# Kamino666/Video-Captioning-Transformer

Hardware: AMD Instinct MI355X
Metric: video-caption train samples/sec (whole node) (higher is better)
Workload: dtype bf16; 1 GPU; configs[1]: 2 enc + 2 dec layers d=512 ff=2048 H=8 V=30522, synthetic (256,12,512) features -> 20-token captions per GPU, fwd+bwd+Adam, dropout 0.3, SCE alpha 0.5; global_batch=256, per_gpu_batch=256, seq_len=20, frames=12, parallelism=dp1, executor=list

## Files before the change

### video-captioning-transformer_amd/csrc/vct_common.h

```cpp
#pragma once
#include <hip/hip_runtime.h>
#include <stdint.h>
#include <utility>
#include <type_traits>
#include "../../include/vct_hip.h"
#include "vct_runtime.h"

namespace vct {

typedef __attribute__((ext_vector_type(4))) uint32_t stream_u32x4;
typedef __attribute__((ext_vector_type(2))) uint32_t stream_u32x2;
__device__ __forceinline__ void store_stream16(void* dst, const stream_u32x4 v) {
  asm volatile("global_store_dwordx4 %0, %1, off sc1" :: "v"(dst), "v"(v) : "memory");
}
__device__ __forceinline__ void store_stream8(void* dst, const stream_u32x2 v) {
  asm volatile("global_store_dwordx2 %0, %1, off sc1" :: "v"(dst), "v"(v) : "memory");
}


typedef __attribute__((ext_vector_type(8))) __bf16 bf16x8;
typedef __attribute__((ext_vector_type(4))) __bf16 bf16x4;
typedef __attribute__((ext_vector_type(4))) short s16x4;
typedef __attribute__((ext_vector_type(8))) short s16x8;
typedef __attribute__((ext_vector_type(4))) float f32x4;
// ... 68 lines not shown
}

struct Dropout {
  uint32_t key;
  uint32_t thresh;
  float scale;
  bool on;
};
__device__ __forceinline__ Dropout make_dropout(const uint32_t* seed, uint32_t site, float p) {
  Dropout d;
  d.on = (seed != nullptr) && (p > 0.0f);
  d.key = d.on ? (seed[0] * 0x9E3779B1u) ^ (site * 0x85EBCA77u + 0x165667B1u) : 0u;
  d.thresh = d.on ? (uint32_t)fminf(p * 65536.0f + 0.5f, 65535.0f) : 0u;
  d.scale = d.on ? 1.0f / (1.0f - p) : 1.0f;
  return d;
}
__device__ __forceinline__ uint32_t hash32(uint32_t x) {
  x ^= x >> 16; x *= 0x85EBCA6Bu; x ^= x >> 13; x *= 0xC2B2AE35u; x ^= x >> 16;
  return x;
}
__device__ __forceinline__ float drop_mult(const Dropout& d, uint32_t idx) {
  if (!d.on) return 1.0f;
  const uint32_t h = hash32(((idx >> 1) * 0x9E3779B1u) ^ d.key);
  const uint32_t f = (idx & 1u) ? (h >> 16) : (h & 0xffffu);
  return f < d.thresh ? 0.0f : d.scale;
}
template <int N> __device__ __forceinline__ void drop_mults(const Dropout& d, uint32_t idx, float (&m)[N]) {
  static_assert(N % 2 == 0, "pairs");
  if (!d.on) {
#pragma unroll
    for (int j = 0; j < N; j++) m[j] = 1.0f;
    return;
  }
  if ((idx & 1u) == 0u) {
#pragma unroll
    for (int k = 0; k < N / 2; k++) {
      const uint32_t h = hash32((((idx >> 1) + (uint32_t)k) * 0x9E3779B1u) ^ d.key);
      m[2 * k] = (h & 0xffffu) < d.thresh ? 0.0f : d.scale;
      m[2 * k + 1] = (h >> 16) < d.thresh ? 0.0f : d.scale;
    }
  } else {
#pragma unroll
    for (int j = 0; j < N; j++) m[j] = drop_mult(d, idx + (uint32_t)j);
  }
}

__device__ __forceinline__ float wave_sum(float v) {
#pragma unroll
  for (int o = 32; o > 0; o >>= 1) v += __shfl_xor(v, o);
  return v;
}
__device__ __forceinline__ float wave_max(float v) {
#pragma unroll
  for (int o = 32; o > 0; o >>= 1) v = fmaxf(v, __shfl_xor(v, o));
  return v;
}
template <int NW> __device__ __forceinline__ float block_sum(float v, float* red) {
  v = wave_sum(v);
  const int w = threadIdx.x >> 6, l = threadIdx.x & 63;
  __syncthreads();
  if (l == 0) red[w] = v;
  __syncthreads();
  float s = 0.0f;
#pragma unroll
  for (int i = 0; i < NW; i++) s += red[i];
  return s;
}
template <int NW> __device__ __forceinline__ float block_max(float v, float* red) {
  v = wave_max(v);
  const int w = threadIdx.x >> 6, l = threadIdx.x & 63;
  __syncthreads();
  if (l == 0) red[w] = v;
  __syncthreads();
  float s = red[0];
#pragma unroll
  for (int i = 1; i < NW; i++) s = fmaxf(s, red[i]);
  return s;
}

__device__ __forceinline__ s16x4 lds_tr16(const bf16_t* p) {
  return __builtin_amdgcn_ds_read_tr16_b64_v4i16((__attribute__((address_space(3))) s16x4*)(p));
}

template <class F, int... Is>
__device__ __forceinline__ void static_for_impl(F&& f, std::integer_sequence<int, Is...>) {
  (f(std::integral_constant<int, Is>{}), ...);
}
template <int N, class F> __device__ __forceinline__ void static_for(F&& f) {
  static_for_impl(static_cast<F&&>(f), std::make_integer_sequence<int, N>{});
}

template <typename T> struct DTypeOf;
template <> struct DTypeOf<float> { static constexpr int v = VCT_F32; };
template <> struct DTypeOf<bf16_t> { static constexpr int v = VCT_BF16; };

}

#define VCT_CHECK_LAUNCH()                               \
  do {                                                   \
    hipError_t e__ = hipGetLastError();                  \
    if (e__ != hipSuccess) return (int)e__;              \
  } while (0)
```

### video-captioning-transformer_amd/csrc/vct_gemm.hip

```cpp
#include <cstdlib>
#include <cstring>
#include "vct_common.h"
#include "vct_gemm_params.h"

namespace vct {

template <typename TI> struct GemmCfg;
template <> struct GemmCfg<float> { static constexpr int BK = 16, VEC = 4, KPAD = 4; };

struct alignas(16) Vec16 { uint32_t w[4]; };
__device__ __forceinline__ Vec16 vec_zero() { Vec16 v; v.w[0] = v.w[1] = v.w[2] = v.w[3] = 0u; return v; }

template <typename TI, bool MC, int R>
struct Stager {
  using Cfg = GemmCfg<TI>;
  static constexpr int BK = Cfg::BK, VEC = Cfg::VEC;
  static constexpr bool BF = sizeof(TI) == 2;
  static constexpr int NV = (R * BK / VEC) / 256;
  static constexpr int KC_STRIDE = BK + Cfg::KPAD;
  static constexpr int LDS_ELEMS = R * KC_STRIDE;
  static_assert(NV >= 1, "tile too small for 256 threads");

  __device__ __forceinline__ static void load(Vec16 (&regs)[NV], const TI* __restrict__ base, long ld, int r0,
                                              int r_ext, int k0, int K) {
// ... 166 lines not shown
      for (int q = 0; q < VO; q += 4) {
        const f32x4 t = *reinterpret_cast<const f32x4*>(stg + rr * STG_STRIDE + cc + q);
        v[q] = t[0]; v[q + 1] = t[1]; v[q + 2] = t[2]; v[q + 3] = t[3];
      }
      if (row >= p.M || col >= p.N) return;
      const bool full = vec_ok && (col + VO <= p.N);
      if (part) {
        float* dst = partC + (size_t)row * p.N + col;
        if (full) {
#pragma unroll
          for (int q = 0; q < VO; q += 4) *reinterpret_cast<f32x4*>(dst + q) = f32x4{v[q], v[q + 1], v[q + 2], v[q + 3]};
        } else {
          for (int q = 0; q < VO; q++) if (col + q < p.N) dst[q] = v[q];
        }
        return;
      }
      if (full) {
        OutV dv, av, ov, pv;
        const bool has_d = dact != nullptr, has_a = addend != nullptr;
        if (has_d) dv = *reinterpret_cast<const OutV*>(dact + (size_t)row * p.ld_dact + col);
        if (has_a) av = *reinterpret_cast<const OutV*>(addend + (size_t)row * p.ld_addend + col);
#pragma unroll
        for (int q = 0; q < VO; q++) {
          float x = v[q] + bvec[c][q];
          pv.e[q] = from_f<TO>(x);
          x = act_f(p.act, x);
          if (has_d) x *= dact_f(p.dact_kind, to_f<TO>(dv.e[q]));
          x *= drop_mult(dr, (uint32_t)row * (uint32_t)p.N + (uint32_t)(col + q));
          if (has_a) x += to_f<TO>(av.e[q]);
          ov.e[q] = from_f<TO>(x);
        }
        *reinterpret_cast<OutV*>(C + (size_t)row * p.ldc + col) = ov;
        if (preact != nullptr) {
          if ((p.ld_preact % VO) == 0) *reinterpret_cast<OutV*>(preact + (size_t)row * p.ld_preact + col) = pv;
          else for (int q = 0; q < VO; q++) preact[(size_t)row * p.ld_preact + col + q] = pv.e[q];
        }
      } else {
        for (int q = 0; q < VO; q++) {
          if (col + q >= p.N) break;
          float x = v[q] + bvec[c][q];
          if (preact != nullptr) preact[(size_t)row * p.ld_preact + col + q] = from_f<TO>(x);
          x = act_f(p.act, x);
          if (dact != nullptr) x *= dact_f(p.dact_kind, to_f<TO>(dact[(size_t)row * p.ld_dact + col + q]));
          x *= drop_mult(dr, (uint32_t)row * (uint32_t)p.N + (uint32_t)(col + q));
          if (addend != nullptr) x += to_f<TO>(addend[(size_t)row * p.ld_addend + col + q]);
          C[(size_t)row * p.ldc + col + q] = from_f<TO>(x);
        }
      }
    });
  });
}

template <typename TO>
__global__ void splitk_reduce_kernel(const float* __restrict__ partial, TO* __restrict__ C, long ldc, int M, int N,
                                     int S, const float* __restrict__ bias_partial, float* __restrict__ bias_grad) {
  const size_t total = (size_t)M * N;
  for (size_t idx = (size_t)blockIdx.x * blockDim.x + threadIdx.x; idx < total; idx += (size_t)gridDim.x * blockDim.x) {
    float s = 0.0f;
    for (int z = 0; z < S; z++) s += partial[(size_t)z * total + idx];
    const int row = (int)(idx / N), col = (int)(idx % N);
    C[(size_t)row * ldc + col] = from_f<TO>(s);
  }
  if (bias_grad != nullptr) {
    for (int row = blockIdx.x * blockDim.x + threadIdx.x; row < M; row += gridDim.x * blockDim.x) {
      float s = 0.0f;
      for (int z = 0; z < S; z++) s += bias_partial[(size_t)z * M + row];
      bias_grad[row] = s;
    }
  }
}

struct Plan { int bm, bn, nbuf, waves8; int split; int tiles_m, tiles_n, nkt, kt_per; };

static bool gemm_can_split(const vct_gemm_desc* d) {
  return d->bias == nullptr && d->act == VCT_ACT_NONE && d->preact == nullptr &&
         d->addend == nullptr && d->dact_src == nullptr && !(d->seed != nullptr && d->p_drop > 0.0f);
}

static bool use_counters(const vct_gemm_desc* d, const Plan& pl) {
  const int64_t partial_bytes = (int64_t)pl.split * d->M * d->N * 4;
  return d->tile_counters != nullptr && d->dtype == VCT_BF16 && (long)pl.tiles_m * pl.tiles_n <= (long)d->n_tile_counters &&
         partial_bytes <= ((int64_t)16 << 20);
}
static Plan gemm_plan(const vct_gemm_desc* d, bool have_ws) {
  Plan pl;
  pl.nbuf = 2;
  pl.waves8 = 0;
  const bool bf = d->dtype == VCT_BF16;
  const int BK = bf ? 64 : 16;
  pl.nkt = (d->K + BK - 1) / BK;
  auto tiles = [&](int bm, int bn) { return (long)((d->M + bm - 1) / bm) * ((d->N + bn - 1) / bn); };
  if (bf) {
    static const int cand[7][2] = {{128, 128}, {128, 64}, {64, 128}, {64, 64}, {256, 128}, {320, 128}, {64, 128}};
    int pick = 3;
    const int rsv = d->reserved >= 99 ? 0 : d->reserved;
    const int tsel = rsv % 10;
    pl.nbuf = (rsv / 10) ? (rsv / 10) : 2;
    const bool cover_ok = d->out_dtype == VCT_BF16 && d->ta == 0;
    if (tsel == 5) { pick = 0; pl.waves8 = 1; }
    else if (tsel == 8) { pick = 1; pl.waves8 = 4; }
    else if (tsel == 6 && cover_ok) { pick = 4; pl.waves8 = 6; pl.nbuf = 2; }
    else if (tsel == 7 && cover_ok) { pick = 5; pl.waves8 = 7; pl.nbuf = 2; }
    else if (tsel == 9 && cover_ok) { pick = 6; pl.waves8 = 9; pl.nbuf = 2; }
    else if (tsel >= 1 && tsel <= 4) pick = tsel - 1;
    else {
      pick = 3;
      static const bool legacy = getenv("VCT_GEMM_4WAVE_ONLY") != nullptr;
      if ((pl.nkt >= 64 && tiles(128, 128) >= 128) || (tiles(64, 64) >= 16384 && d->N >= 4096)) {
        pick = 0; pl.waves8 = legacy ? 0 : 1;
        if (legacy && pl.nkt < 64) pick = 2;
      } else if (!legacy && d->N >= 1024 && d->M >= 2048 && pl.nkt <= 16) { pick = 1; pl.waves8 = 4; }
    }
    pl.bm = cand[pick][0]; pl.bn = cand[pick][1];
  } else {
    pl.bm = pl.bn = (tiles(128, 128) >= 384) ? 128 : 64;
  }
  pl.tiles_m = (d->M + pl.bm - 1) / pl.bm;
  pl.tiles_n = (d->N + pl.bn - 1) / pl.bn;
  const long nt = (long)pl.tiles_m * pl.tiles_n;
  int split = 1;
  if (d->split_k > 1) split = d->split_k;
  else if (d->split_k == 0 && nt < 384 && pl.nkt >= 8) split = (int)((767 + nt) / nt);
  const bool epilogue = !gemm_can_split(d);
  if (!have_ws || (epilogue && (d->tile_counters == nullptr || !bf))) split = 1;
  if (epilogue && d->split_k == 0 && d->M > 16) split = 1;
  if (split > pl.nkt / 2) split = pl.nkt / 2 > 0 ? pl.nkt / 2 : 1;
  if (split < 1) split = 1;
  pl.kt_per = (pl.nkt + split - 1) / split;
  pl.split = (pl.nkt + pl.kt_per - 1) / pl.kt_per;
  if ((epilogue || d->adam != nullptr) && pl.split > 1 && !use_counters(d, pl)) { pl.split = 1; pl.kt_per = pl.nkt; }
  return pl;
}

template <typename TI, typename TO, int TA, int TB, int BM>
static void launch_gemm(const GemmP& p, dim3 grid, hipStream_t st) {
  vct::launch((gemm_kernel<TI, TO, TA, TB, BM, BM>), grid, dim3(256), 0, st, p);
}

template <typename TI, typename TO>
static int dispatch_layout(const vct_gemm_desc* d, const GemmP& p, int bm, dim3 grid, hipStream_t st) {
  const int key = d->ta * 2 + d->tb;
#define VCT_L(TA_, TB_)                                              \
  if (bm == 128) launch_gemm<TI, TO, TA_, TB_, 128>(p, grid, st);    \
  else launch_gemm<TI, TO, TA_, TB_, 64>(p, grid, st);               \
  return VCT_OK;
  switch (key) {
    case 1: { VCT_L(0, 1) }
    case 0: { VCT_L(0, 0) }
    case 2: { VCT_L(1, 0) }
    default: return VCT_E_SHAPE;
  }
#undef VCT_L
}

int gemm_bf16_v2_dispatch(const vct_gemm_desc* d, const GemmP& p, int bm, int bn, int nbuf, dim3 grid, hipStream_t st);
int gemm256_try(const vct_gemm_desc* d, hipStream_t st, bool* used, int* reduce_split);
int gemm_skinny_try(const vct_gemm_desc* d, hipStream_t st, bool* used);
int gemm_pt_try(const vct_gemm_desc* d, hipStream_t st, bool* used);

}

using namespace vct;

static int64_t ws_bytes(const vct_gemm_desc* d, const Plan& pl) {
  if (pl.split <= 1) return 0;
  return (int64_t)pl.split * ((int64_t)d->M * d->N + d->M) * 4;
}

extern "C" int64_t vct_gemm_workspace_bytes(const vct_gemm_desc* d) {
  if (d == nullptr) return 0;
  return ws_bytes(d, gemm_plan(d, true));
}

static int check_desc(const vct_gemm_desc* d) {
  if (d == nullptr || d->A == nullptr || d->B == nullptr || d->C == nullptr) return VCT_E_ARG;
  if (d->dtype != VCT_F32 && d->dtype != VCT_BF16) return VCT_E_ARG;
  if (d->out_dtype != VCT_F32 && d->out_dtype != VCT_BF16) return VCT_E_ARG;
  if (d->M <= 0 || d->N <= 0 || d->K <= 0) return VCT_E_SHAPE;
  if (d->ta == 1 && d->tb == 1) return VCT_E_SHAPE;
  const int vec = d->dtype == VCT_BF16 ? 8 : 4;
  if (d->lda % vec || d->ldb % vec) return VCT_E_ALIGN;
  if (((uintptr_t)d->A & 15) || ((uintptr_t)d->B & 15)) return VCT_E_ALIGN;
  if (d->dact_src != nullptr && d->act == VCT_ACT_NONE) return VCT_E_ARG;
  if (d->bias_grad != nullptr && d->dtype == VCT_BF16 && !(d->ta == 1 && d->tb == 0 && d->out_dtype == VCT_F32)) return VCT_E_ARG;
  if (d->adam != nullptr) {
    const vct_gemm_adam* a = d->adam;
    if (!(d->dtype == VCT_BF16 && d->out_dtype == VCT_F32 && d->ta == 1 && d->tb == 0)) return VCT_E_ARG;
    if (d->bias != nullptr || d->act != VCT_ACT_NONE || d->preact != nullptr || d->addend != nullptr || d->dact_src != nullptr ||
        (d->seed != nullptr && d->p_drop > 0.0f))
      return VCT_E_ARG;
    if (!a->param || !a->exp_avg || !a->exp_avg_sq || !a->hyper || !a->step) return VCT_E_ARG;
    if (((uintptr_t)a->param | (uintptr_t)a->exp_avg | (uintptr_t)a->exp_avg_sq | (uintptr_t)d->C) & 15) return VCT_E_ALIGN;
    if (d->ldc % 4) return VCT_E_ALIGN;
    if (a->shadow != nullptr && (((uintptr_t)a->shadow & 7) || (a->ld_shadow % 4))) return VCT_E_ALIGN;
    if (a->pk_stream != nullptr && (a->shadow == nullptr || ((uintptr_t)a->pk_stream & 15) || a->pk_K < d->N || (a->pk_K % 8) ||
                                    a->pk_row0 < 0 || (a->pk_mode != 0 && a->pk_mode != 1)))
      return VCT_E_ARG;
    if (a->pk_stream != nullptr)
      for (int i = 0; i < 4; i++) if (a->pk_chunk0[i] >= 0xffff) return VCT_E_ARG;
  }
  return VCT_OK;
}

static void fill_params(const vct_gemm_desc* d, const Plan& pl, GemmP& p) {
  p.A = d->A; p.B = d->B; p.C = d->C;
  p.lda = d->lda; p.ldb = d->ldb; p.ldc = d->ldc;
  p.M = d->M; p.N = d->N; p.K = d->K;
  p.kt_per_split = pl.kt_per;
  p.tiles_m = pl.tiles_m;
  p.tiles_n = pl.tiles_n;
  p.act = d->dact_src != nullptr ? VCT_ACT_NONE : d->act;
  p.dact_kind = d->dact_src != nullptr ? d->act : VCT_ACT_NONE;
  p.bias = d->bias;
  p.preact = d->preact; p.ld_preact = d->ld_preact;
  p.addend = d->addend; p.ld_addend = d->ld_addend;
  p.dact = d->dact_src; p.ld_dact = d->ld_dact;
  p.seed = d->seed; p.site = d->site; p.p_drop = d->p_drop;
  p.bias_grad = d->bias_grad;
  p.partial = nullptr; p.bias_partial = nullptr; p.counters = nullptr;
  memset(&p.adam, 0, sizeof(p.adam));
  if (d->adam != nullptr) {
    const vct_gemm_adam* a = d->adam;
    p.adam.param = a->param; p.adam.m = a->exp_avg; p.adam.v = a->exp_avg_sq;
    p.adam.shadow = reinterpret_cast<uint16_t*>(a->shadow); p.adam.ld_shadow = (long)a->ld_shadow;
    p.adam.pk_stream = reinterpret_cast<uint16_t*>(a->pk_stream); p.adam.pk_K = a->pk_K; p.adam.pk_mode = a->pk_mode;
    {
      auto f = [](int c) { return (unsigned long long)(c < 0 || c >= 0xffff ? 0xffff : c); };
      p.adam.pk_chunks = f(a->pk_chunk0[0]) | (f(a->pk_chunk0[1]) << 16) | (f(a->pk_chunk0[2]) << 32) | (f(a->pk_chunk0[3]) << 48);
    }
    p.adam.pk_row0 = a->pk_row0; p.adam.store_grad = a->store_grad;
    p.adam.hyper = a->hyper; p.adam.step = a->step;
  }
  p.waves8 = pl.waves8;
  p.split = pl.split;
  {
    static const char* env = getenv("VCT_GEMM_NT");
    p.nt_store = env != nullptr ? atoi(env) : 0;
  }
  {
    static const char* env = getenv("VCT_GEMM_NT_PREACT");
    p.nt_preact = env != nullptr ? (env[0] == '1') : 0;
  }
  {
    static const char* env = getenv("VCT_GEMM_ORDER");
    const int ts = pl.tiles_m < pl.tiles_n ? pl.tiles_m : pl.tiles_n;
    p.short_fast = env != nullptr ? (env[0] == '1') : (pl.split > 1 && ts <= 4);
  }
  if (pl.split > 1) {
    if (use_counters(d, pl)) p.counters = d->tile_counters;
    p.partial = reinterpret_cast<float*>(d->workspace);
    p.bias_partial = p.partial + (size_t)pl.split * d->M * d->N;
  }
}

extern "C" int vct_gemm(const vct_gemm_desc* d, void* stream) {
  const int ok = check_desc(d);
  if (ok != VCT_OK) return ok;
  hipStream_t st = (hipStream_t)stream;
  const bool general_only = d->adam != nullptr;
  if (!general_only) {
    bool used = false;
    const int rcs = gemm_skinny_try(d, st, &used);
    if (rcs != VCT_OK || used) return rcs;
  }
  if (!general_only || (d->ta == 1 && d->tb == 0)) {
    bool used = false;
    int rsplit = 1;
    const int rc256 = gemm256_try(d, st, &used, &rsplit);
    if (rc256 != VCT_OK) return rc256;
    if (used) {
      if (rsplit > 1) {
        const size_t total = (size_t)d->M * d->N;
        const int blocks = (int)((total + 255) / 256 < 2048 ? (total + 255) / 256 : 2048);
        vct::launch((splitk_reduce_kernel<bf16_t>), dim3(blocks), dim3(256), 0, st, reinterpret_cast<const float*>(d->workspace),
                    reinterpret_cast<bf16_t*>(d->C), (long)d->ldc, d->M, d->N, rsplit, (const float*)nullptr, (float*)nullptr);
        VCT_CHECK_LAUNCH();
      }
      return VCT_OK;
    }
  }

  if (!general_only) {
    bool used = false;
    const int rcp = gemm_pt_try(d, st, &used);
    if (rcp != VCT_OK || used) return rcp;
  }

  const int64_t need = vct_gemm_workspace_bytes(d);
  const bool have_ws = d->workspace != nullptr && d->workspace_bytes >= need && need > 0;
  if (d->split_k > 1 && !have_ws) return VCT_E_WORKSPACE;
  const Plan pl = gemm_plan(d, have_ws);

  GemmP p;
  fill_params(d, pl, p);
  const dim3 grid(pl.tiles_m * pl.tiles_n, 1, pl.split);
  int rc;
  if (d->dtype == VCT_BF16) {
    rc = gemm_bf16_v2_dispatch(d, p, pl.bm, pl.bn, pl.nbuf, grid, st);
  } else {
    if (d->out_dtype != VCT_F32) return VCT_E_ARG;
    rc = dispatch_layout<float, float>(d, p, pl.bm, grid, st);
  }
  if (rc != VCT_OK) return rc;
  VCT_CHECK_LAUNCH();
  if (pl.split > 1 && p.counters == nullptr) {
    const size_t total = (size_t)d->M * d->N;
    const int blocks = (int)((total + 255) / 256 < 2048 ? (total + 255) / 256 : 2048);
    if (d->out_dtype == VCT_F32)
      vct::launch((splitk_reduce_kernel<float>), dim3(blocks), dim3(256), 0, st, p.partial,
                         reinterpret_cast<float*>(d->C), (long)d->ldc, d->M, d->N, pl.split, p.bias_partial, d->bias_grad);
    else
      vct::launch((splitk_reduce_kernel<bf16_t>), dim3(blocks), dim3(256), 0, st, p.partial,
                         reinterpret_cast<bf16_t*>(d->C), (long)d->ldc, d->M, d->N, pl.split, p.bias_partial, d->bias_grad);
    VCT_CHECK_LAUNCH();
  }
  return VCT_OK;
}

namespace vct {
int gemm_bf16_v2_grouped_tn(const GemmGroupP& g, int bm, int bn, int total_wg, hipStream_t st);
}

struct GroupTile { int bm, bn, waves8; };
static long group_tiles(const vct_gemm_desc* descs, int n, const GroupTile& t) {
  long gt = 0;
  for (int k = 0; k < n; k++) gt += (long)((descs[k].M + t.bm - 1) / t.bm) * ((descs[k].N + t.bn - 1) / t.bn);
  return gt;
}
static GroupTile grouped_tile(const vct_gemm_desc* descs, int n) {
  static const int env_sel = [] { const char* e = getenv("VCT_GROUP_TILE"); return e ? atoi(e) : 0; }();
  const int sel = descs[0].reserved % 10 ? descs[0].reserved % 10 : env_sel;
  if (sel == 4) return GroupTile{64, 64, 0};
  if (sel == 8) return GroupTile{128, 64, 4};
  if (sel == 5) return GroupTile{128, 128, 1};
  const GroupTile big{128, 128, 1};
  return group_tiles(descs, n, big) >= 160 ? big : GroupTile{64, 64, 0};
}
static Plan grouped_plan(const vct_gemm_desc* d, const GroupTile& t, long gt) {
  Plan pl;
  pl.bm = t.bm; pl.bn = t.bn; pl.nbuf = 2; pl.waves8 = t.waves8;
  pl.nkt = (d->K + 63) / 64;
  pl.tiles_m = (d->M + t.bm - 1) / t.bm;
  pl.tiles_n = (d->N + t.bn - 1) / t.bn;
  int split = gt >= 192 ? 1 : (int)((255 + gt) / gt);
  if (d->split_k >= 1) split = d->split_k;
  if (split > pl.nkt / 4) split = pl.nkt / 4 > 0 ? pl.nkt / 4 : 1;
  while (split > 1 && (int64_t)split * d->M * d->N * 4 > ((int64_t)16 << 20)) split--;
  if (split < 1) split = 1;
  pl.kt_per = (pl.nkt + split - 1) / split;
  pl.split = (pl.nkt + pl.kt_per - 1) / pl.kt_per;
  return pl;
}

extern "C" int64_t vct_gemm_grouped_workspace_bytes(const vct_gemm_desc* descs, int32_t n, int32_t i) {
  if (descs == nullptr || n < 1 || n > VCT_GEMM_GROUP_MAX || i < 0 || i >= n) return 0;
  const GroupTile t = grouped_tile(descs, n);
  return ws_bytes(descs + i, grouped_plan(descs + i, t, group_tiles(descs, n, t)));
}

extern "C" int vct_gemm_grouped(const vct_gemm_desc* descs, int32_t n, void* stream) {
  if (descs == nullptr || n < 1 || n > VCT_GEMM_GROUP_MAX) return VCT_E_ARG;
  for (int i = 0; i < n; i++) {
    const vct_gemm_desc* d = descs + i;
    const int ok = check_desc(d);
    if (ok != VCT_OK) return ok;
    if (d->dtype != VCT_BF16 || d->out_dtype != VCT_F32 || d->ta != 1 || d->tb != 0 || !gemm_can_split(d)) return VCT_E_ARG;
  }
  const GroupTile t = grouped_tile(descs, n);
  const long gt = group_tiles(descs, n, t);
  GemmGroupP g;
  g.n = n;
  int wg = 0;
  static const bool group_map_on = [] { const char* e = getenv("VCT_GROUP_MAP"); return !(e && e[0] == '0'); }();
  bool group_map = group_map_on;
  for (int i = 0; i < n && group_map; i++) group_map = grouped_plan(descs + i, t, gt).split == 1;
  for (int i = 0; i < n; i++) {
    const vct_gemm_desc* d = descs + i;
    const Plan pl = grouped_plan(d, t, gt);
    if (pl.split > 1) {
      if (!use_counters(d, pl)) return VCT_E_WORKSPACE;
      if (d->workspace == nullptr || d->workspace_bytes < ws_bytes(d, pl)) return VCT_E_WORKSPACE;
    }
    fill_params(d, pl, g.p[i]);
    g.start[i] = wg;
    wg += group_map ? pl.tiles_m * pl.tiles_n : (pl.tiles_m * pl.tiles_n * pl.split + 7) & ~7;
  }
  g.total = group_map ? wg : 0;
  for (int i = n; i < VCT_GEMM_GROUP_MAX; i++) { g.start[i] = wg; g.p[i] = g.p[0]; }
  wg = (wg + 7) & ~7;
  const int rc = gemm_bf16_v2_grouped_tn(g, t.bm, t.bn, wg, (hipStream_t)stream);
  if (rc != VCT_OK) return rc;
  VCT_CHECK_LAUNCH();
  return VCT_OK;
}
```

### video-captioning-transformer_amd/csrc/vct_gemm_bf16_kernel.h

```cpp
#pragma once
#include <type_traits>
#ifndef VCT_GEMM_DMA_IL
#define VCT_GEMM_DMA_IL(TA, TB, BM, BN, NW) ((TA) == 0 && (TB) == 0)
#endif
#include "vct_common.h"
#include "vct_adam_core.h"
#include "vct_gemm_params.h"

namespace vct {

constexpr int BK2 = 64;

__device__ __forceinline__ int kc_off(int row, int chunk) { return row * 128 + ((chunk ^ (row & 7)) << 4); }
template <int R> __device__ __forceinline__ int mc_off(int krow, int col) {
  constexpr int NB = R / 16;
  const int b = col >> 4;
  return krow * (R * 2) + (((b ^ (krow & (NB - 1))) << 5) | ((col & 15) << 1));
}

template <bool MC, int R, int NW>
__device__ __forceinline__ void dma_tile(unsigned char* lds, const bf16_t* __restrict__ base, long ld, int r0, int r_ext,
                                         int k0, int wave, int lane) {
  constexpr int NI = R * 8 / (64 * NW);
  static_assert(NI >= 1, "tile too small for this many waves");
// ... 190 lines not shown

  const bf16_t* A = reinterpret_cast<const bf16_t*>(p.A);
  const bf16_t* B = reinterpret_cast<const bf16_t*>(p.B);

  f32x4 acc[TM][TN];
  constexpr int TMB = (TM + WGN - 1) / WGN;
  f32x4 accb[TMB];
#pragma unroll
  for (int u = 0; u < TMB; u++) accb[u] = f32x4{0, 0, 0, 0};
#pragma unroll
  for (int i = 0; i < TM; i++) {
#pragma unroll
    for (int j = 0; j < TN; j++) acc[i][j] = f32x4{0, 0, 0, 0};
  }
  constexpr bool BG = (TA == 1 && TB == 0 && sizeof(TO) == 4);
  const bool do_bias_grad = BG && (p.bias_grad != nullptr) && (tile_n == 0);
  const s16x8 ones_s = {0x3F80, 0x3F80, 0x3F80, 0x3F80, 0x3F80, 0x3F80, 0x3F80, 0x3F80};
  const bf16x8 ones = __builtin_bit_cast(bf16x8, ones_s);

  auto compute = [&](const unsigned char* la, const unsigned char* lb, auto WITH_DMA, unsigned char* nb, const int ktn) {
    constexpr bool DMA = decltype(WITH_DMA)::value;
    constexpr int KS = BK2 / 32;
    bf16x8 fa[KS][TM], fb[KS][TN];
#pragma unroll
    for (int ks = 0; ks < KS; ks++) {
#pragma unroll
      for (int i = 0; i < TM; i++) fa[ks][i] = frag2<A_MC, BM, KSPLIT>(la, wm * WM + i * 16, ks, lane);
#pragma unroll
      for (int j = 0; j < TN; j++) fb[ks][j] = frag2<B_MC, BN, KSPLIT>(lb, wn * WN + j * 16, ks, lane);
    }
#pragma unroll
    for (int ks = 0; ks < KS; ks++)
#pragma unroll
      for (int i = 0; i < TM; i++)
#pragma unroll
        for (int j = 0; j < TN; j++) acc[i][j] = __builtin_amdgcn_mfma_f32_16x16x32_bf16(fa[ks][i], fb[ks][j], acc[i][j], 0, 0, 0);
    constexpr int N_DSREAD = KS * (TM * (A_MC ? 2 : 1) + TN * (B_MC ? 2 : 1));
    constexpr int NMF = KS * TM * TN;
    if constexpr (DMA) {
      constexpr int NP = BM * 8 / (64 * NW) + BN * 8 / (64 * NW);
      constexpr int GRP = (NMF / 2 / NP) > 0 ? (NMF / 2 / NP) : 1;
      dma_tile<A_MC, BM, NW>(nb, A, p.lda, m0, p.M, ktn * BK2, wave, lane);
      dma_tile<B_MC, BN, NW>(nb + A_BYTES, B, p.ldb, n0, p.N, ktn * BK2, wave, lane);
      __builtin_amdgcn_sched_group_barrier(0x100, N_DSREAD, 0);
      static_for<NP>([&](auto) {
        __builtin_amdgcn_sched_group_barrier(0x008, GRP, 0);
        __builtin_amdgcn_sched_group_barrier(0x020, 1, 0);
      });
      if constexpr (NMF - NP * GRP > 0) __builtin_amdgcn_sched_group_barrier(0x008, NMF - NP * GRP, 0);
    } else {
      __builtin_amdgcn_sched_group_barrier(0x100, N_DSREAD, 0);
      __builtin_amdgcn_sched_group_barrier(0x008, NMF, 0);
    }
    if constexpr (BG) {
      if (do_bias_grad) {
        static_for<TM>([&](auto I) {
          constexpr int i = decltype(I)::value;
          if (wn == i % WGN) {
#pragma unroll
            for (int ks = 0; ks < KS; ks++) accb[i / WGN] = __builtin_amdgcn_mfma_f32_16x16x32_bf16(fa[ks][i], ones, accb[i / WGN], 0, 0, 0);
          }
        });
      }
    }
  };

  auto stage = [&](int kt, int buf) {
    unsigned char* nb = lds_raw + buf * BUF_BYTES;
    if (kt < kt_full_end) {
      dma_tile<A_MC, BM, NW>(nb, A, p.lda, m0, p.M, kt * BK2, wave, lane);
      dma_tile<B_MC, BN, NW>(nb + A_BYTES, B, p.ldb, n0, p.N, kt * BK2, wave, lane);
    } else {
      tail_tile<A_MC, BM, NT>(nb, A, p.lda, m0, p.M, kt * BK2, p.K, tid);
      tail_tile<B_MC, BN, NT>(nb + A_BYTES, B, p.ldb, n0, p.N, kt * BK2, p.K, tid);
    }
  };
  if constexpr (NBUF == 1) {
    for (int kt = kt_begin; kt < kt_end; kt++) {
      if (kt > kt_begin) __syncthreads();
      stage(kt, 0);
      __syncthreads();
      compute(lds_raw, lds_raw + A_BYTES, std::false_type{}, nullptr, 0);
    }
  } else {
    static_assert(NBUF == 2, "NBUF is 1 or 2");
    if (kt_begin < kt_end) stage(kt_begin, 0);
    int cur = 0;
    int kt = kt_begin;
    if constexpr (DMA_IL) {
      for (; kt + 1 < kt_full_end; kt++) {
        __syncthreads();
        const unsigned char* la = lds_raw + cur * BUF_BYTES;
        compute(la, la + A_BYTES, std::true_type{}, lds_raw + (cur ^ 1) * BUF_BYTES, kt + 1);
        cur ^= 1;
      }
    }
    for (; kt < kt_end; kt++) {
      __syncthreads();
      if (kt + 1 < kt_end) stage(kt + 1, cur ^ 1);
      compute(lds_raw + cur * BUF_BYTES, lds_raw + cur * BUF_BYTES + A_BYTES, std::false_type{}, nullptr, 0);
      cur ^= 1;
    }
  }

  const int c16 = lane & 15, g4 = (lane >> 4) * 4;
  if (do_bias_grad && c16 == 0) {
    float* bg = p.partial != nullptr ? p.bias_partial + (size_t)zid * p.M : p.bias_grad;
#pragma unroll
    for (int u = 0; u < TMB; u++)
#pragma unroll
      for (int r = 0; r < 4; r++) {
        const int i = wn + u * WGN;
        const int row = m0 + wm * WM + i * 16 + g4 + r;
        if (i < TM && row < p.M) {
          if (p.counters != nullptr) coherent_store1(bg + row, accb[u][r]);
          else bg[row] = accb[u][r];
        }
      }
  }
  __syncthreads();
  float* stage_base = reinterpret_cast<float*>(lds_raw);
  constexpr int VO = 16 / (int)sizeof(TO);
  constexpr bool SLAB = (BM * BN != 128 * 128);
  constexpr int SLAB_ROWS = WGM * 16, CPRW = BN / VO;
  constexpr int CPRV = WN / VO;
  constexpr int SSTR = SLAB ? BN + 4 : WN + 4;
  constexpr int STAGE_FLOATS = SLAB ? SLAB_ROWS * SSTR : NW * 16 * SSTR;
  constexpr int NSLAB = (SLAB && 2 * STAGE_FLOATS * 4 <= NBUF * BUF_BYTES) ? 2 : 1;
  static_assert(STAGE_FLOATS * 4 <= NBUF * BUF_BYTES, "epilogue staging must fit in the operand buffers");
  static_assert(!SLAB || (SLAB_ROWS * CPRW) % NT == 0, "slab chunks must divide over the workgroup");
  constexpr int CPL = SLAB ? SLAB_ROWS * CPRW / NT : (16 * CPRV + 63) / 64;
  const bool part = p.partial != nullptr;
  int e_lds[CPL], e_row[CPL], e_col[CPL];
  bool e_act[CPL];
  float bvec[CPL][VO];
#pragma unroll
  for (int c = 0; c < CPL; c++) {
    if constexpr (SLAB) {
      const int chunk = c * NT + tid;
      const int sr = chunk / CPRW, sc = (chunk % CPRW) * VO;
      e_lds[c] = sr * SSTR + sc; e_row[c] = (sr >> 4) * WM + (sr & 15); e_col[c] = sc; e_act[c] = true;
    } else {
      const int chunk = c * 64 + lane;
      const int rr = (chunk / CPRV) & 15, cc = (chunk % CPRV) * VO;
      e_lds[c] = wave * 16 * SSTR + rr * SSTR + cc; e_row[c] = wm * WM + rr; e_col[c] = wn * WN + cc;
      e_act[c] = chunk < 16 * CPRV;
    }
#pragma unroll
    for (int q = 0; q < VO; q++) bvec[c][q] = 0.0f;
  }
  if (p.bias != nullptr && (!part || p.counters != nullptr)) {
#pragma unroll
    for (int c = 0; c < CPL; c++) {
#pragma unroll
      for (int q = 0; q < VO; q++) bvec[c][q] = p.bias[min(n0 + e_col[c] + q, p.N - 1)];
    }
  }

  const Dropout dr = make_dropout(p.seed, p.site, p.p_drop);
  TO* C = reinterpret_cast<TO*>(p.C);
  TO* preact = reinterpret_cast<TO*>(p.preact);
  const TO* addend = reinterpret_cast<const TO*>(p.addend);
  const TO* dact = reinterpret_cast<const TO*>(p.dact);
  float* partC = part ? p.partial + (size_t)zid * (size_t)p.M * (size_t)p.N : nullptr;
  const long ldo = part ? (long)p.N : p.ldc;
  const bool vec_ok = (ldo % VO == 0) && (part || (((uintptr_t)p.C & 15) == 0));
// ... 160 lines not shown
      const int row = m0 + e_row[c] + i * 16, col = n0 + e_col[c];
      float v[VO];
#pragma unroll
      for (int q = 0; q < VO; q += 4) {
        const f32x4 t = *reinterpret_cast<const f32x4*>(stage + e_lds[c] + q);
        v[q] = t[0]; v[q + 1] = t[1]; v[q + 2] = t[2]; v[q + 3] = t[3];
      }
      if (!e_act[c]) return;
      if (row >= p.M || col >= p.N) return;
      const bool full = vec_ok && (col + VO <= p.N);
      if (part) {
        float* dst = partC + (size_t)row * p.N + col;
        if (p.counters != nullptr) {
          if (full) {
#pragma unroll
            for (int q = 0; q < VO; q += 2) coherent_store2(dst + q, v[q], v[q + 1]);
          } else {
            for (int q = 0; q < VO; q++) if (col + q < p.N) coherent_store1(dst + q, v[q]);
          }
        } else if (full) {
#pragma unroll
          for (int q = 0; q < VO; q += 4) *reinterpret_cast<f32x4*>(dst + q) = f32x4{v[q], v[q + 1], v[q + 2], v[q + 3]};
        } else {
          for (int q = 0; q < VO; q++) if (col + q < p.N) dst[q] = v[q];
        }
        return;
      }
      finish(row, col, v, bvec[c], full, adam_direct ? &areg[c] : nullptr);
    });
  });

  if (part && p.counters != nullptr) {
    __shared__ int s_last;
    asm volatile("s_waitcnt vmcnt(0)" ::: "memory");
    __syncthreads();
    if (tid == 0)
      s_last = (__hip_atomic_fetch_add(p.counters + wgid, 1, __ATOMIC_RELAXED, __HIP_MEMORY_SCOPE_AGENT) == p.split - 1) ? 1 : 0;
    __syncthreads();
    if (!s_last) return;
    const size_t zstride = (size_t)p.M * (size_t)p.N;
    static_for<TM>([&](auto I) {
      constexpr int i = decltype(I)::value;
      static_for<CPL>([&](auto CI) {
        constexpr int c = decltype(CI)::value;
        const int row = m0 + e_row[c] + i * 16, col = n0 + e_col[c];
        if (!e_act[c] || row >= p.M || col >= p.N) return;
        const float* src = p.partial + (size_t)row * p.N + col;
        const bool full = vec_ok && (col + VO <= p.N) && (p.ldc % VO == 0) && (((uintptr_t)p.C & 15) == 0);
        float s[VO];
#pragma unroll
        for (int q = 0; q < VO; q++) s[q] = 0.0f;
        if (full) {
          for (int z = 0; z < p.split; z++) {
#pragma unroll
            for (int q = 0; q < VO; q += 2) {
              float t0, t1;
              coherent_load2(src + (size_t)z * zstride + q, t0, t1);
              s[q] += t0; s[q + 1] += t1;
            }
          }
        } else {
          for (int q = 0; q < VO; q++) {
            if (col + q >= p.N) break;
            for (int z = 0; z < p.split; z++) s[q] += coherent_load1(src + (size_t)z * zstride + q);
          }
        }
        finish(row, col, s, bvec[c], full, nullptr);
      });
    });
    if (p.bias_grad != nullptr && tile_n == 0) {
      for (int r = tid; r < BM; r += NT) {
        const int row = m0 + r;
        if (row < p.M) {
          float a = 0.0f;
          for (int z = 0; z < p.split; z++) a += coherent_load1(p.bias_partial + (size_t)z * p.M + row);
          p.bias_grad[row] = a;
        }
      }
    }
    if (tid == 0) __hip_atomic_store(p.counters + wgid, 0, __ATOMIC_RELAXED, __HIP_MEMORY_SCOPE_AGENT);
  }
}

constexpr int gemm_min_waves(int bm, int bn, int nw) { return nw == 8 ? (bm * bn == 128 * 128 ? 4 : (bm * bn == 128 * 64 ? 6 : 1)) : 1; }

template <typename TO, int TA, int TB, int BM, int BN, int NBUF, int WGM = 2, int WGN = 2>
__global__ __launch_bounds__(64 * WGM * WGN, gemm_min_waves(BM, BN, WGM * WGN)) void gemm_bf16_v2_kernel(const GemmP p) {
  gemm_bf16_v2_body<TO, TA, TB, BM, BN, NBUF, WGM, WGN>(p, blockIdx.x, blockIdx.z);
}

template <typename TO, int TA, int TB, int BM, int BN, int NBUF, int WGM, int WGN>
__global__ __launch_bounds__(64 * WGM * WGN, gemm_min_waves(BM, BN, WGM * WGN)) void gemm_bf16_v2_grouped_kernel(const GemmGroupP g) {
  const int b = blockIdx.x;
  int at = b;
  const bool direct = g.total > 0;
  if (direct) {
    const int xcd = b & 7, slot = b >> 3;
    const int q = g.total >> 3, r = g.total & 7;
    if (slot >= q + (xcd < r ? 1 : 0)) return;
    at = (xcd < r ? xcd * (q + 1) : r * (q + 1) + (xcd - r) * q) + slot;
  }
  int gi = 0;
#pragma unroll
  for (int i = 1; i < VCT_GEMM_GROUP_MAX; i++) gi = (i < g.n && at >= g.start[i]) ? i : gi;
  const GemmP& p = g.p[gi];
  const int local = at - g.start[gi], nwg = p.tiles_m * p.tiles_n;
  if (local >= nwg * p.split) return;
  gemm_bf16_v2_body<TO, TA, TB, BM, BN, NBUF, WGM, WGN>(p, local % nwg, local / nwg, direct);
}

template <typename TO, int TA, int TB, int NBUF>
static int launch_tiles(const GemmP& p, int bm, int bn, dim3 grid, hipStream_t st) {
#define VCT_LAUNCH(BM_, BN_) vct::launch((gemm_bf16_v2_kernel<TO, TA, TB, BM_, BN_, NBUF>), grid, dim3(256), 0, st, p)
  if (p.waves8) {
#define VCT_LW(BM_, BN_, WM_, WN_) vct::launch((gemm_bf16_v2_kernel<TO, TA, TB, BM_, BN_, NBUF, WM_, WN_>), grid, dim3(64 * WM_ * WN_), 0, st, p)
    if (p.waves8 == 1 && bm == 128 && bn == 128) VCT_LW(128, 128, 2, 4);
    else if (p.waves8 == 4 && bm == 128 && bn == 64) VCT_LW(128, 64, 4, 2);
    else if constexpr (sizeof(TO) == 2 && TA == 0 && NBUF == 2) {
      if (p.waves8 == 6 && bm == 256 && bn == 128) VCT_LW(256, 128, 4, 2);
      else if (p.waves8 == 7 && bm == 320 && bn == 128) VCT_LW(320, 128, 4, 2);
      else if (p.waves8 == 9 && bm == 64 && bn == 128) VCT_LW(64, 128, 2, 4);
      else return VCT_E_SHAPE;
    }
    else return VCT_E_SHAPE;
#undef VCT_LW
  }
  else if (bm == 128 && bn == 128) VCT_LAUNCH(128, 128);
  else if (bm == 128 && bn == 64) VCT_LAUNCH(128, 64);
  else if (bm == 64 && bn == 128) VCT_LAUNCH(64, 128);
  else if (bm == 64 && bn == 64) VCT_LAUNCH(64, 64);
  else return VCT_E_SHAPE;
#undef VCT_LAUNCH
  return VCT_OK;
}

template <typename TO, int TA, int TB>
static int launch_nbuf(const GemmP& p, int bm, int bn, int nbuf, dim3 grid, hipStream_t st) {
  if (nbuf == 1) return launch_tiles<TO, TA, TB, 1>(p, bm, bn, grid, st);
  return launch_tiles<TO, TA, TB, 2>(p, bm, bn, grid, st);
}


template <int TA, int TB>
static int gemm_bf16_v2_layout(const vct_gemm_desc* d, const GemmP& p, int bm, int bn, int nbuf, dim3 grid, hipStream_t st) {
  return d->out_dtype == VCT_BF16 ? launch_nbuf<bf16_t, TA, TB>(p, bm, bn, nbuf, grid, st)
                                  : launch_nbuf<float, TA, TB>(p, bm, bn, nbuf, grid, st);
}

}
```

### video-captioning-transformer_amd/csrc/vct_gemm_bf16_tn.hip

```cpp
#include "vct_gemm_bf16_kernel.h"
namespace vct {
int gemm_bf16_v2_tn(const vct_gemm_desc* d, const GemmP& p, int bm, int bn, int nbuf, dim3 grid, hipStream_t st) {
  return gemm_bf16_v2_layout<1, 0>(d, p, bm, bn, nbuf, grid, st);
}
int gemm_bf16_v2_grouped_tn(const GemmGroupP& g, int bm, int bn, int total_wg, hipStream_t st) {
  if (bm == 128 && bn == 128)
    vct::launch((gemm_bf16_v2_grouped_kernel<float, 1, 0, 128, 128, 2, 2, 4>), dim3(total_wg), dim3(512), 0, st, g);
  else if (bm == 128 && bn == 64)
    vct::launch((gemm_bf16_v2_grouped_kernel<float, 1, 0, 128, 64, 2, 4, 2>), dim3(total_wg), dim3(512), 0, st, g);
  else if (bm == 64 && bn == 64)
    vct::launch((gemm_bf16_v2_grouped_kernel<float, 1, 0, 64, 64, 2, 2, 2>), dim3(total_wg), dim3(256), 0, st, g);
  else
    return VCT_E_SHAPE;
  return VCT_OK;
}
}
```

### video-captioning-transformer_amd/csrc/vct_gemm_params.h

```cpp
#pragma once
#include <stdint.h>
#include "../../include/vct_hip.h"

namespace vct {

struct AdamEpiP {
  float* param; float* m; float* v;
  uint16_t* shadow; long ld_shadow;
  uint16_t* pk_stream; int pk_K, pk_mode; int pk_row0; int store_grad;
  unsigned long long pk_chunks;
  const float* hyper; const int32_t* step;
};

struct GemmP {
  const void* A; const void* B; void* C;
  long lda, ldb, ldc;
  int M, N, K;
  int kt_per_split;
  int tiles_m, tiles_n;
  int act;
  int dact_kind;
  const float* bias;
  void* preact; long ld_preact;
  const void* addend; long ld_addend;
  const void* dact; long ld_dact;
  const uint32_t* seed; uint32_t site; float p_drop;
  float* bias_grad;
  float* partial;
  float* bias_partial;
  int waves8;
  int split;
  int* counters;
  int nt_store;
  int nt_preact;
  int short_fast;
  AdamEpiP adam;
};

struct GemmGroupP {
  int n;
  int total;
  int start[VCT_GEMM_GROUP_MAX];
  GemmP p[VCT_GEMM_GROUP_MAX];
};

}
```

Measured before the change: 123,500 samples/s.

## Add three-slot LDS ring pipeline for selected bf16 GEMM shapes

Adds an NBUF=3 main loop to the bf16 GEMM kernel. Global-to-LDS staging runs two k-tiles ahead, LDS fragment reads use inline asm with immediate offsets, and explicit vmcnt/lgkmcnt waits let the second k-step's reads overlap the first k-step's MFMAs. The planner switches the default-enabled form (mask 2: NN bf16 64x64 tiles with kt_per >= 4) to the ring, and the grouped TN path can opt in through a mask. The ring uses more LDS per block and lowers launch-bounds occupancy hints, so fewer blocks may fit per CU. An env-controlled dynamic-LDS padding probe is also added, off by default.

```diff
diff --git a/video-captioning-transformer_amd/csrc/vct_common.h b/video-captioning-transformer_amd/csrc/vct_common.h
--- a/video-captioning-transformer_amd/csrc/vct_common.h
+++ b/video-captioning-transformer_amd/csrc/vct_common.h
@@ -174,6 +174,28 @@
   return __builtin_amdgcn_ds_read_tr16_b64_v4i16((__attribute__((address_space(3))) s16x4*)(p));
 }
 
+template <int OFF> __device__ __forceinline__ s16x4 lds_tr16_asm(uint32_t ad) {
+  static_assert(OFF >= 0 && OFF < 65536, "ds offset field is 16 bits");
+  s16x4 v;
+  asm volatile("ds_read_b64_tr_b16 %0, %1 offset:%2" : "=v"(v) : "v"(ad), "n"(OFF) : "memory");
+  return v;
+}
+template <int OFF> __device__ __forceinline__ s16x8 lds_b128_asm(uint32_t ad) {
+  static_assert(OFF >= 0 && OFF < 65536, "ds offset field is 16 bits");
+  s16x8 v;
+  asm volatile("ds_read_b128 %0, %1 offset:%2" : "=v"(v) : "v"(ad), "n"(OFF) : "memory");
+  return v;
+}
+template <typename V> __device__ __forceinline__ void lds_asm_tie(V& v) { asm volatile("" : "+v"(v)); }
+template <int N> __device__ __forceinline__ void wait_vmcnt() {
+  static_assert(N >= 0 && N < 64, "vmcnt is 6 bits");
+  asm volatile("s_waitcnt vmcnt(%0)" :: "n"(N) : "memory");
+}
+template <int N> __device__ __forceinline__ void wait_lgkmcnt() {
+  static_assert(N >= 0 && N < 16, "lgkmcnt is 4 bits");
+  asm volatile("s_waitcnt lgkmcnt(%0)" :: "n"(N) : "memory");
+}
+
 template <class F, int... Is>
 __device__ __forceinline__ void static_for_impl(F&& f, std::integer_sequence<int, Is...>) {
   (f(std::integral_constant<int, Is>{}), ...);
diff --git a/video-captioning-transformer_amd/csrc/vct_gemm.hip b/video-captioning-transformer_amd/csrc/vct_gemm.hip
--- a/video-captioning-transformer_amd/csrc/vct_gemm.hip
+++ b/video-captioning-transformer_amd/csrc/vct_gemm.hip
@@ -272,6 +272,16 @@
   return d->tile_counters != nullptr && d->dtype == VCT_BF16 && (long)pl.tiles_m * pl.tiles_n <= (long)d->n_tile_counters &&
          partial_bytes <= ((int64_t)16 << 20);
 }
+#ifndef VCT_GEMM_RING_DEFAULT
+#define VCT_GEMM_RING_DEFAULT 2
+#endif
+static int gemm_ring_mask() {
+  const char* e = getenv("VCT_GEMM_RING");
+  return e != nullptr ? atoi(e) : VCT_GEMM_RING_DEFAULT;
+}
+constexpr int GEMM_RING_MIN_KT = 4;
+static bool gemm_ring_auto(int form, int kt_per) { return form != 0 && kt_per >= GEMM_RING_MIN_KT && (gemm_ring_mask() & form) != 0; }
+
 static Plan gemm_plan(const vct_gemm_desc* d, bool have_ws) {
   Plan pl;
   pl.nbuf = 2;
@@ -319,6 +329,9 @@
   pl.kt_per = (pl.nkt + split - 1) / split;
   pl.split = (pl.nkt + pl.kt_per - 1) / pl.kt_per;
   if ((epilogue || d->adam != nullptr) && pl.split > 1 && !use_counters(d, pl)) { pl.split = 1; pl.kt_per = pl.nkt; }
+  if (bf && pl.nbuf == 2 && (d->reserved >= 99 ? 0 : d->reserved) / 10 == 0 &&
+      gemm_ring_auto(gemm_ring_form(d->ta, d->tb, d->out_dtype, pl.bm, pl.bn, pl.waves8), pl.kt_per))
+    pl.nbuf = 3;
   return pl;
 }
 
@@ -424,6 +437,11 @@
   p.waves8 = pl.waves8;
   p.split = pl.split;
   {
+    const char* env = getenv("VCT_GEMM_PAD_LDS");
+    const int pad = env != nullptr ? atoi(env) : 0;
+    p.pad_lds = (pad > 0 && pad <= 32768 && pl.nbuf != 3) ? pad : 0;
+  }
+  {
     static const char* env = getenv("VCT_GEMM_NT");
     p.nt_store = env != nullptr ? atoi(env) : 0;
   }
@@ -508,7 +526,7 @@
 }
 
 namespace vct {
-int gemm_bf16_v2_grouped_tn(const GemmGroupP& g, int bm, int bn, int total_wg, hipStream_t st);
+int gemm_bf16_v2_grouped_tn(const GemmGroupP& g, int bm, int bn, int nbuf, int total_wg, hipStream_t st);
 }
 
 struct GroupTile { int bm, bn, waves8; };
@@ -578,7 +596,16 @@
   g.total = group_map ? wg : 0;
   for (int i = n; i < VCT_GEMM_GROUP_MAX; i++) { g.start[i] = wg; g.p[i] = g.p[0]; }
   wg = (wg + 7) & ~7;
-  const int rc = gemm_bf16_v2_grouped_tn(g, t.bm, t.bn, wg, (hipStream_t)stream);
+  int nbuf = 2;
+  const int rsv_nbuf = descs[0].reserved / 10;
+  if (rsv_nbuf == 3) nbuf = 3;
+  else if (rsv_nbuf == 0) {
+    const int form = gemm_ring_form(1, 0, VCT_F32, t.bm, t.bn, t.waves8);
+    bool ring = form != 0 && (gemm_ring_mask() & form) != 0;
+    for (int i = 0; i < n && ring; i++) ring = g.p[i].kt_per_split >= GEMM_RING_MIN_KT;
+    if (ring) nbuf = 3;
+  }
+  const int rc = gemm_bf16_v2_grouped_tn(g, t.bm, t.bn, nbuf, wg, (hipStream_t)stream);
   if (rc != VCT_OK) return rc;
   VCT_CHECK_LAUNCH();
   return VCT_OK;
diff --git a/video-captioning-transformer_amd/csrc/vct_gemm_bf16_kernel.h b/video-captioning-transformer_amd/csrc/vct_gemm_bf16_kernel.h
--- a/video-captioning-transformer_amd/csrc/vct_gemm_bf16_kernel.h
+++ b/video-captioning-transformer_amd/csrc/vct_gemm_bf16_kernel.h
@@ -296,6 +296,124 @@
       __syncthreads();
       compute(lds_raw, lds_raw + A_BYTES, std::false_type{}, nullptr, 0);
     }
+  } else if constexpr (NBUF == 3) {
+    constexpr int KS = BK2 / 32;
+    static_assert(KS == 2, "two k-steps per stage");
+    constexpr int NP = BM * 8 / (64 * NW) + BN * 8 / (64 * NW);
+    constexpr int NRD = TM * (A_MC ? 2 : 1) + TN * (B_MC ? 2 : 1);
+    static_assert(NRD <= 15, "the k-step-1 reads are counted in lgkmcnt (4 bits)");
+    static_assert(!A_MC || KSPLIT || BM <= 64, "second transpose read of A must keep the swizzle");
+    static_assert(!B_MC || KSPLIT || BN <= 64, "second transpose read of B must keep the swizzle");
+    static_assert(BUF_BYTES % 128 == 0 && A_BYTES % 128 == 0, "slot bases keep address bit 6");
+    constexpr int A_HI = (KSPLIT ? 16 : 4) * BM * 2, B_HI = (KSPLIT ? 16 : 4) * BN * 2;
+    constexpr int A_KS = 32 * BM * 2, B_KS = 32 * BN * 2;
+    const uint32_t lds0 = (uint32_t)(uintptr_t)(__attribute__((address_space(3))) unsigned char*)lds_raw;
+    const int fi = lane & 15, fg = lane >> 4;
+    uint32_t offA[A_MC ? TM : 1], offB[B_MC ? TN : 1];
+    if constexpr (A_MC) {
+#pragma unroll
+      for (int i = 0; i < TM; i++) offA[i] = (uint32_t)mc_off<BM>((KSPLIT ? fg * 4 : fg * 8) + (fi >> 2), wm * WM + i * 16 + (fi & 3) * 4);
+    } else {
+      offA[0] = (uint32_t)kc_off(wm * WM + fi, fg);
+    }
+    if constexpr (B_MC) {
+#pragma unroll
+      for (int j = 0; j < TN; j++)
+        offB[j] = (uint32_t)(A_BYTES + mc_off<BN>((KSPLIT ? fg * 4 : fg * 8) + (fi >> 2), wn * WN + j * 16 + (fi & 3) * 4));
+    } else {
+      offB[0] = (uint32_t)(A_BYTES + kc_off(wn * WN + fi, fg));
+    }
+    s16x4 pa[KS][TM][2], pb[KS][TN][2];
+    s16x8 qa[KS][TM], qb[KS][TN];
+    auto read_step = [&](auto KSI, const uint32_t sb) {
+      constexpr int ks = decltype(KSI)::value;
+      static_for<TM>([&](auto I) {
+        constexpr int i = decltype(I)::value;
+        if constexpr (A_MC) {
+          pa[ks][i][0] = lds_tr16_asm<ks * A_KS>(sb + offA[i]);
+          pa[ks][i][1] = lds_tr16_asm<ks * A_KS + A_HI>(sb + offA[i]);
+        } else {
+          qa[ks][i] = lds_b128_asm<i * 2048>((sb + offA[0]) ^ (uint32_t)(ks * 64));
+        }
+      });
+      static_for<TN>([&](auto J) {
+        constexpr int j = decltype(J)::value;
+        if constexpr (B_MC) {
+          pb[ks][j][0] = lds_tr16_asm<ks * B_KS>(sb + offB[j]);
+          pb[ks][j][1] = lds_tr16_asm<ks * B_KS + B_HI>(sb + offB[j]);
+        } else {
+          qb[ks][j] = lds_b128_asm<j * 2048>((sb + offB[0]) ^ (uint32_t)(ks * 64));
+        }
+      });
+    };
+    bf16x8 fa[KS][TM], fb[KS][TN];
+    auto take_step = [&](auto KSI) {
+      constexpr int ks = decltype(KSI)::value;
+#pragma unroll
+      for (int i = 0; i < TM; i++) {
+        if constexpr (A_MC) {
+          lds_asm_tie(pa[ks][i][0]); lds_asm_tie(pa[ks][i][1]);
+          const s16x4 lo = pa[ks][i][0], hi = pa[ks][i][1];
+          const s16x8 v = {lo[0], lo[1], lo[2], lo[3], hi[0], hi[1], hi[2], hi[3]};
+          fa[ks][i] = __builtin_bit_cast(bf16x8, v);
+        } else {
+          lds_asm_tie(qa[ks][i]);
+          fa[ks][i] = __builtin_bit_cast(bf16x8, qa[ks][i]);
+        }
+      }
+#pragma unroll
+      for (int j = 0; j < TN; j++) {
+        if constexpr (B_MC) {
+          lds_asm_tie(pb[ks][j][0]); lds_asm_tie(pb[ks][j][1]);
+          const s16x4 lo = pb[ks][j][0], hi = pb[ks][j][1];
+          const s16x8 v = {lo[0], lo[1], lo[2], lo[3], hi[0], hi[1], hi[2], hi[3]};
+          fb[ks][j] = __builtin_bit_cast(bf16x8, v);
+        } else {
+          lds_asm_tie(qb[ks][j]);
+          fb[ks][j] = __builtin_bit_cast(bf16x8, qb[ks][j]);
+        }
+      }
+    };
+    if (kt_begin < kt_end) stage(kt_begin, 0);
+    if (kt_begin + 1 < kt_end) stage(kt_begin + 1, 1);
+    int cur = 0;
+    for (int kt = kt_begin; kt < kt_end; kt++) {
+      if (kt + 1 < kt_full_end) wait_vmcnt<NP>();
+      else wait_vmcnt<0>();
+      lds_barrier();
+      const int fre = cur == 0 ? 2 : cur - 1;
+      const int kt2 = kt + 2;
+      if (kt2 < kt_end) stage(kt2, fre);
+      const uint32_t sb = lds0 + (uint32_t)(cur * BUF_BYTES);
+      read_step(std::integral_constant<int, 0>{}, sb);
+      read_step(std::integral_constant<int, 1>{}, sb);
+      wait_lgkmcnt<NRD>();
+      take_step(std::integral_constant<int, 0>{});
+      static_for<TM * TN>([&](auto MI) {
+        constexpr int m = decltype(MI)::value, i = m / TN, j = m % TN;
+        acc[i][j] = __builtin_amdgcn_mfma_f32_16x16x32_bf16(fa[0][i], fb[0][j], acc[i][j], 0, 0, 0);
+      });
+      __builtin_amdgcn_sched_barrier(0);
+      wait_lgkmcnt<0>();
+      take_step(std::integral_constant<int, 1>{});
+      static_for<TM * TN>([&](auto MI) {
+        constexpr int m = decltype(MI)::value, i = m / TN, j = m % TN;
+        acc[i][j] = __builtin_amdgcn_mfma_f32_16x16x32_bf16(fa[1][i], fb[1][j], acc[i][j], 0, 0, 0);
+      });
+      if constexpr (BG) {
+        if (do_bias_grad) {
+          static_for<TM>([&](auto I) {
+            constexpr int i = decltype(I)::value;
+            if (wn == i % WGN) {
+#pragma unroll
+              for (int ks = 0; ks < KS; ks++) accb[i / WGN] = __builtin_amdgcn_mfma_f32_16x16x32_bf16(fa[ks][i], ones, accb[i / WGN], 0, 0, 0);
+            }
+          });
+        }
+      }
+      cur = cur == 2 ? 0 : cur + 1;
+    }
+    asm volatile("s_waitcnt vmcnt(0) lgkmcnt(0)" ::: "memory");
   } else {
     static_assert(NBUF == 2, "NBUF is 1 or 2");
     if (kt_begin < kt_end) stage(kt_begin, 0);
@@ -622,15 +740,18 @@
   }
 }
 
-constexpr int gemm_min_waves(int bm, int bn, int nw) { return nw == 8 ? (bm * bn == 128 * 128 ? 4 : (bm * bn == 128 * 64 ? 6 : 1)) : 1; }
+constexpr int gemm_min_waves(int bm, int bn, int nw, int nbuf = 2) {
+  if (nbuf == 3) return nw == 8 ? (bm * bn == 128 * 128 ? 2 : (bm * bn == 128 * 64 ? 4 : 1)) : 1;
+  return nw == 8 ? (bm * bn == 128 * 128 ? 4 : (bm * bn == 128 * 64 ? 6 : 1)) : 1;
+}
 
 template <typename TO, int TA, int TB, int BM, int BN, int NBUF, int WGM = 2, int WGN = 2>
-__global__ __launch_bounds__(64 * WGM * WGN, gemm_min_waves(BM, BN, WGM * WGN)) void gemm_bf16_v2_kernel(const GemmP p) {
+__global__ __launch_bounds__(64 * WGM * WGN, gemm_min_waves(BM, BN, WGM * WGN, NBUF)) void gemm_bf16_v2_kernel(const GemmP p) {
   gemm_bf16_v2_body<TO, TA, TB, BM, BN, NBUF, WGM, WGN>(p, blockIdx.x, blockIdx.z);
 }
 
 template <typename TO, int TA, int TB, int BM, int BN, int NBUF, int WGM, int WGN>
-__global__ __launch_bounds__(64 * WGM * WGN, gemm_min_waves(BM, BN, WGM * WGN)) void gemm_bf16_v2_grouped_kernel(const GemmGroupP g) {
+__global__ __launch_bounds__(64 * WGM * WGN, gemm_min_waves(BM, BN, WGM * WGN, NBUF)) void gemm_bf16_v2_grouped_kernel(const GemmGroupP g) {
   const int b = blockIdx.x;
   int at = b;
   const bool direct = g.total > 0;
@@ -651,7 +772,7 @@
 
 template <typename TO, int TA, int TB, int NBUF>
 static int launch_tiles(const GemmP& p, int bm, int bn, dim3 grid, hipStream_t st) {
-#define VCT_LAUNCH(BM_, BN_) vct::launch((gemm_bf16_v2_kernel<TO, TA, TB, BM_, BN_, NBUF>), grid, dim3(256), 0, st, p)
+#define VCT_LAUNCH(BM_, BN_) vct::launch((gemm_bf16_v2_kernel<TO, TA, TB, BM_, BN_, NBUF>), grid, dim3(256), (size_t)p.pad_lds, st, p)
   if (p.waves8) {
 #define VCT_LW(BM_, BN_, WM_, WN_) vct::launch((gemm_bf16_v2_kernel<TO, TA, TB, BM_, BN_, NBUF, WM_, WN_>), grid, dim3(64 * WM_ * WN_), 0, st, p)
     if (p.waves8 == 1 && bm == 128 && bn == 128) VCT_LW(128, 128, 2, 4);
@@ -675,7 +796,28 @@
 }
 
 template <typename TO, int TA, int TB>
+static int launch_ring(const GemmP& p, int bm, int bn, dim3 grid, hipStream_t st) {
+  if constexpr (TA == 1 && TB == 0 && sizeof(TO) == 4) {
+    if (bm == 128 && bn == 128 && p.waves8 == 1) {
+      vct::launch((gemm_bf16_v2_kernel<TO, TA, TB, 128, 128, 3, 2, 4>), grid, dim3(512), 0, st, p);
+      return VCT_OK;
+    }
+  } else if constexpr (TA == 0 && TB == 0 && sizeof(TO) == 2) {
+    if (bm == 64 && bn == 64 && p.waves8 == 0) {
+      vct::launch((gemm_bf16_v2_kernel<TO, TA, TB, 64, 64, 3, 2, 2>), grid, dim3(256), 0, st, p);
+      return VCT_OK;
+    }
+    if (bm == 128 && bn == 64 && p.waves8 == 4) {
+      vct::launch((gemm_bf16_v2_kernel<TO, TA, TB, 128, 64, 3, 4, 2>), grid, dim3(512), 0, st, p);
+      return VCT_OK;
+    }
+  }
+  return VCT_E_SHAPE;
+}
+
+template <typename TO, int TA, int TB>
 static int launch_nbuf(const GemmP& p, int bm, int bn, int nbuf, dim3 grid, hipStream_t st) {
+  if (nbuf == 3) return launch_ring<TO, TA, TB>(p, bm, bn, grid, st);
   if (nbuf == 1) return launch_tiles<TO, TA, TB, 1>(p, bm, bn, grid, st);
   return launch_tiles<TO, TA, TB, 2>(p, bm, bn, grid, st);
 }
diff --git a/video-captioning-transformer_amd/csrc/vct_gemm_bf16_tn.hip b/video-captioning-transformer_amd/csrc/vct_gemm_bf16_tn.hip
--- a/video-captioning-transformer_amd/csrc/vct_gemm_bf16_tn.hip
+++ b/video-captioning-transformer_amd/csrc/vct_gemm_bf16_tn.hip
@@ -3,8 +3,14 @@
 int gemm_bf16_v2_tn(const vct_gemm_desc* d, const GemmP& p, int bm, int bn, int nbuf, dim3 grid, hipStream_t st) {
   return gemm_bf16_v2_layout<1, 0>(d, p, bm, bn, nbuf, grid, st);
 }
-int gemm_bf16_v2_grouped_tn(const GemmGroupP& g, int bm, int bn, int total_wg, hipStream_t st) {
-  if (bm == 128 && bn == 128)
+int gemm_bf16_v2_grouped_tn(const GemmGroupP& g, int bm, int bn, int nbuf, int total_wg, hipStream_t st) {
+  if (nbuf == 3) {
+    if (bm == 128 && bn == 128)
+      vct::launch((gemm_bf16_v2_grouped_kernel<float, 1, 0, 128, 128, 3, 2, 4>), dim3(total_wg), dim3(512), 0, st, g);
+    else
+      return VCT_E_SHAPE;
+  }
+  else if (bm == 128 && bn == 128)
     vct::launch((gemm_bf16_v2_grouped_kernel<float, 1, 0, 128, 128, 2, 2, 4>), dim3(total_wg), dim3(512), 0, st, g);
   else if (bm == 128 && bn == 64)
     vct::launch((gemm_bf16_v2_grouped_kernel<float, 1, 0, 128, 64, 2, 4, 2>), dim3(total_wg), dim3(512), 0, st, g);
diff --git a/video-captioning-transformer_amd/csrc/vct_gemm_params.h b/video-captioning-transformer_amd/csrc/vct_gemm_params.h
--- a/video-captioning-transformer_amd/csrc/vct_gemm_params.h
+++ b/video-captioning-transformer_amd/csrc/vct_gemm_params.h
@@ -33,9 +33,17 @@
   int* counters;
   int nt_store;
   int nt_preact;
+  int pad_lds;
   int short_fast;
   AdamEpiP adam;
 };
+
+static inline int gemm_ring_form(int ta, int tb, int out_dtype, int bm, int bn, int waves8) {
+  if (ta == 1 && tb == 0 && out_dtype == VCT_F32) return (bm == 128 && bn == 128 && waves8 == 1) ? 1 : 0;
+  if (ta == 0 && tb == 0 && out_dtype == VCT_BF16)
+    return (bm == 64 && bn == 64 && waves8 == 0) ? 2 : ((bm == 128 && bn == 64 && waves8 == 4) ? 4 : 0);
+  return 0;
+}
 
 struct GemmGroupP {
   int n;
```

Result: no change. 124,600 samples/s, median of 6 (+0.9%).
